# ai4co/rl4co

Hardware: NVIDIA H100
Metric: node-selections/sec TSP-100 AM rollout (higher is better)
Workload: dtype f32

## Files before the change

rl4co_b200/csrc/gemm_tf32x3.cu:

```cuda
#include "co_common.cuh"
#include "wgmma.cuh"

namespace co {

constexpr int GM = 128, GN = 128, GK = 32;
constexpr int TILE_BYTES = GM * GK * 4;
constexpr uint32_t SBO = 1024;
constexpr int KB128 = 4;
constexpr int STAGES = 3;
constexpr int GEMM_THREADS = 384;
constexpr int GEMM_SMEM = 2 * KB128 * TILE_BYTES + STAGES * 2 * TILE_BYTES;

__device__ __forceinline__ float4 split_hi(float4 v) {
  return make_float4(wg::rna_tf32(v.x), wg::rna_tf32(v.y), wg::rna_tf32(v.z), wg::rna_tf32(v.w));
}
__device__ __forceinline__ float4 sub4(float4 a, float4 b) { return make_float4(a.x - b.x, a.y - b.y, a.z - b.z, a.w - b.w); }

__global__ void split_tf32_kernel(const float* __restrict__ w, float* __restrict__ hi, float* __restrict__ lo, long n) {
  long i = (long)blockIdx.x * blockDim.x + threadIdx.x;
  if (i < n) {
    const float v = w[i], h = wg::rna_tf32(v);
    hi[i] = h;
    lo[i] = v - h;
  }
}

struct GemmArgs {
  const float* A; const float* Whi; const float* Wlo; float* C;
  const float* bias; const float* residual; const float* scale; const float* shift;
  int M, Nout, K, lda, ldc, ldr, relu, n_tiles;
};

__device__ __forceinline__ void epilogue_regs(const GemmArgs& g, const float (&d)[64], int m0, int n0, int lane) {
  const int q = lane & 3;
#pragma unroll
  for (int j = 0; j < 16; ++j) {
    const int n = n0 + 8 * j + 2 * q;
    if (n >= g.Nout) continue;
    float2 bs = make_float2(0.f, 0.f), sc = make_float2(1.f, 1.f), sh = bs;
    if (g.bias) bs = __ldg(reinterpret_cast<const float2*>(g.bias + n));
    if (g.scale) { sc = __ldg(reinterpret_cast<const float2*>(g.scale + n)); sh = __ldg(reinterpret_cast<const float2*>(g.shift + n)); }
#pragma unroll
    for (int half = 0; half < 2; ++half) {
      const int row = m0 + (lane >> 2) + 8 * half;
      if (row >= g.M) continue;
      float2 o = make_float2(d[4 * j + 2 * half] + bs.x, d[4 * j + 2 * half + 1] + bs.y);
      if (g.residual) {
        const float2 r = *reinterpret_cast<const float2*>(g.residual + (size_t)row * g.ldr + n);
        o.x += r.x; o.y += r.y;
      }
      if (g.relu) { o.x = fmaxf(o.x, 0.f); o.y = fmaxf(o.y, 0.f); }
      if (g.scale) { o.x = fmaf(o.x, sc.x, sh.x); o.y = fmaf(o.y, sc.y, sh.y); }
      *reinterpret_cast<float2*>(g.C + (size_t)row * g.ldc + n) = o;
    }
  }
}

template <bool WSTAT>
struct KBlock {
  float4 a[8];
  float4 h[WSTAT ? 1 : 8], l[WSTAT ? 1 : 8];
};

template <bool WSTAT>
__global__ void __launch_bounds__(GEMM_THREADS, 1) gemm_tf32x3_kernel(const GemmArgs g, int m_tiles, int groups) {
  extern __shared__ __align__(1024) unsigned char smem[];
  constexpr int STAGE_BYTES = (WSTAT ? 2 : 4) * TILE_BYTES;
  unsigned char* sW = smem;
  unsigned char* sRing = smem + (WSTAT ? 2 * KB128 * TILE_BYTES : 0);
  __shared__ __align__(8) uint64_t bars[2 * STAGES];

  const int tid = threadIdx.x, warp = tid >> 5, lane = tid & 31;
  const int n_tile = blockIdx.x % g.n_tiles, group = blockIdx.x / g.n_tiles;
  const int n0 = n_tile * GN;
  const int nkb = g.K / GK;
  const uint32_t bar0 = wg::s32(bars);
  auto FULL_B = [&](int s) { return bar0 + 8 * s; };
  auto EMPTY_B = [&](int s) { return bar0 + 8 * (STAGES + s); };

  if (tid == 0) {
    for (int s = 0; s < STAGES; ++s) { wg::bar_init(FULL_B(s), 128); wg::bar_init(EMPTY_B(s), 256); }
    wg::bar_init_fence();
  }
  if (WSTAT) {
    const int r8 = lane & 7, c4 = lane >> 3;
    for (int item = warp; item < KB128 * 32; item += GEMM_THREADS / 32) {
      const int kb = item >> 5, qq = item & 31;
      const int rg = qq >> 1, chunk = 4 * (qq & 1) + c4, row = 8 * rg + r8;
      const uint32_t soff = rg * SBO + r8 * 128 + ((chunk ^ r8) << 4);
      float4 h = make_float4(0.f, 0.f, 0.f, 0.f), l = h;
      if (n0 + row < g.Nout) {
        h = __ldg(reinterpret_cast<const float4*>(g.Whi + (size_t)(n0 + row) * g.K + kb * GK + chunk * 4));
        l = __ldg(reinterpret_cast<const float4*>(g.Wlo + (size_t)(n0 + row) * g.K + kb * GK + chunk * 4));
      }
      *reinterpret_cast<float4*>(sW + (2 * kb) * TILE_BYTES + soff) = h;
      *reinterpret_cast<float4*>(sW + (2 * kb + 1) * TILE_BYTES + soff) = l;
    }
    wg::fence_async();
  }
  __syncthreads();

  if (warp < 4) {
    const int r4 = lane >> 3, c8 = lane & 7;
    auto load = [&](int mt, int kb, auto& R) {
#pragma unroll
      for (int j = 0; j < 8; ++j) {
        const int lrow = 16 * j + 4 * warp + r4;
        const int row = mt * GM + lrow;
        R.a[j] = make_float4(0.f, 0.f, 0.f, 0.f);
        if (mt < m_tiles && row < g.M)
          R.a[j] = __ldg(reinterpret_cast<const float4*>(g.A + (size_t)row * g.lda + kb * GK + c8 * 4));
        if constexpr (!WSTAT) {
          R.h[j] = R.l[j] = make_float4(0.f, 0.f, 0.f, 0.f);
          if (mt < m_tiles && n0 + lrow < g.Nout) {
            R.h[j] = __ldg(reinterpret_cast<const float4*>(g.Whi + (size_t)(n0 + lrow) * g.K + kb * GK + c8 * 4));
            R.l[j] = __ldg(reinterpret_cast<const float4*>(g.Wlo + (size_t)(n0 + lrow) * g.K + kb * GK + c8 * 4));
          }
        }
      }
    };
    KBlock<WSTAT> R;
    KBlock<true> Rn;
    load(group, 0, R);
    uint32_t it = 0;
    for (int mt = group; mt < m_tiles; mt += groups) {
      for (int kb = 0; kb < nkb; ++kb, ++it) {
        auto load_next = [&](auto& dst) { if (kb + 1 < nkb) load(mt, kb + 1, dst); else load(mt + groups, 0, dst); };
        if constexpr (WSTAT) load_next(Rn);
        const int s = it % STAGES;
        wg::bar_wait(EMPTY_B(s), ((it / STAGES) & 1) ^ 1);
        unsigned char* st = sRing + s * STAGE_BYTES;
#pragma unroll
        for (int j = 0; j < 8; ++j) {
          const int lrow = 16 * j + 4 * warp + r4;
          const uint32_t soff = (lrow >> 3) * SBO + (lrow & 7) * 128 + ((c8 ^ (lrow & 7)) << 4);
          const float4 h = split_hi(R.a[j]);
          *reinterpret_cast<float4*>(st + soff) = h;
          *reinterpret_cast<float4*>(st + TILE_BYTES + soff) = sub4(R.a[j], h);
          if (!WSTAT) {
            *reinterpret_cast<float4*>(st + 2 * TILE_BYTES + soff) = R.h[j];
            *reinterpret_cast<float4*>(st + 3 * TILE_BYTES + soff) = R.l[j];
          }
        }
        wg::fence_async();
        wg::bar_arrive(FULL_B(s));
        if constexpr (WSTAT) R = Rn; else load_next(R);
      }
    }
  } else {
    const int cw = (warp - 4) >> 2, w4 = warp & 3;
    uint32_t it = 0;
    float d[64];
    for (int mt = group; mt < m_tiles; mt += groups) {
      for (int kb = 0; kb < nkb; ++kb, ++it) {
        const int s = it % STAGES;
        wg::bar_wait(FULL_B(s), (it / STAGES) & 1);
        const uint32_t ahi = wg::s32(sRing + s * STAGE_BYTES) + cw * 64 * 128, alo = ahi + TILE_BYTES;
        const uint32_t bhi = WSTAT ? wg::s32(sW + (2 * kb) * TILE_BYTES) : wg::s32(sRing + s * STAGE_BYTES + 2 * TILE_BYTES);
        const uint32_t blo = bhi + TILE_BYTES;
        wg::pin(d);
        wg::fence();
#pragma unroll
        for (int kk = 0; kk < GK / 8; ++kk) {
          const uint32_t off = kk * 32;
          wg::mma_ss_n128(d, wg::desc_sw128(ahi + off, SBO), wg::desc_sw128(bhi + off, SBO), (kb | kk) != 0);
          wg::mma_ss_n128(d, wg::desc_sw128(alo + off, SBO), wg::desc_sw128(bhi + off, SBO), 1);
          wg::mma_ss_n128(d, wg::desc_sw128(ahi + off, SBO), wg::desc_sw128(blo + off, SBO), 1);
        }
        wg::commit();
        if (kb > 0) {
          wg::wait<1>();
          wg::bar_arrive(EMPTY_B((it - 1) % STAGES));
        }
      }
      wg::wait<0>();
      wg::pin(d);
      wg::bar_arrive(EMPTY_B((it - 1) % STAGES));
      epilogue_regs(g, d, mt * GM + 64 * cw + 16 * w4, n0, lane);
    }
  }
}

}

using namespace co;

extern "C" int co_split_tf32(const float* w, float* hi, float* lo, long n, void* stream) {
  if (!w || !hi || !lo || n < 0) return fail(CO_ERR_BAD_ARG, "co_split_tf32: bad argument%s");
  if (n == 0) return CO_OK;
  split_tf32_kernel<<<(unsigned)((n + 255) / 256), 256, 0, (cudaStream_t)stream>>>(w, hi, lo, n);
  return check_launch("co_split_tf32");
}

extern "C" int co_gemm_tf32x3(const float* A, const float* Whi, const float* Wlo, float* C, const float* bias,
                              const float* residual, const float* scale, const float* shift, int M, int Nout, int K,
                              int lda, int ldc, int ldr, int relu, void* stream) {
  if (!A || !Whi || !Wlo || !C) return fail(CO_ERR_BAD_ARG, "co_gemm_tf32x3: null pointer%s");
  if (M < 0 || Nout <= 0 || K <= 0) return fail(CO_ERR_BAD_ARG, "co_gemm_tf32x3: bad shape%s");
  if ((K % GK) || (Nout % 4) || (lda % 4) || (ldc % 4) || (residual && (ldr % 4)))
    return fail(CO_ERR_UNSUPPORTED, "co_gemm_tf32x3: K %% 32, Nout %% 4 and 16-byte row strides required%s");
  if ((scale == nullptr) != (shift == nullptr)) return fail(CO_ERR_BAD_ARG, "co_gemm_tf32x3: scale and shift go together%s");
  if (((uintptr_t)A | (uintptr_t)Whi | (uintptr_t)Wlo | (uintptr_t)C | (uintptr_t)bias | (uintptr_t)residual |
       (uintptr_t)scale | (uintptr_t)shift) & 15)
    return fail(CO_ERR_BAD_ARG, "co_gemm_tf32x3: pointers must be 16-byte aligned%s");
  if (M == 0) return CO_OK;
  GemmArgs g{A, Whi, Wlo, C, bias, residual, scale, shift, M, Nout, K, lda, ldc, ldr, relu, (Nout + GN - 1) / GN};
  const int m_tiles = (M + GM - 1) / GM;
  if ((long)m_tiles * g.n_tiles > 0x7fffffffL) return fail(CO_ERR_UNSUPPORTED, "co_gemm_tf32x3: too many tiles%s");
  static PerDeviceOnce once;
  bool& configured = once.flag();
  if (!configured) {
    cudaError_t e = cudaFuncSetAttribute(gemm_tf32x3_kernel<true>, cudaFuncAttributeMaxDynamicSharedMemorySize, GEMM_SMEM);
    if (e == cudaSuccess)
      e = cudaFuncSetAttribute(gemm_tf32x3_kernel<false>, cudaFuncAttributeMaxDynamicSharedMemorySize, STAGES * 4 * TILE_BYTES);
    if (e != cudaSuccess) return fail(CO_ERR_CUDA, "co_gemm_tf32x3: smem attribute: %s", cudaGetErrorString(e));
    configured = true;
  }
  int groups = device_info().sm_count / g.n_tiles;
  if (groups < 1) groups = 1;
  if (groups > m_tiles) groups = m_tiles;
  if (K == GK * KB128)
    gemm_tf32x3_kernel<true><<<groups * g.n_tiles, GEMM_THREADS, GEMM_SMEM, (cudaStream_t)stream>>>(g, m_tiles, groups);
  else
    gemm_tf32x3_kernel<false><<<groups * g.n_tiles, GEMM_THREADS, STAGES * 4 * TILE_BYTES, (cudaStream_t)stream>>>(g, m_tiles, groups);
  return check_launch("co_gemm_tf32x3");
}
```

Baseline: 109.0 million.

## Overlap previous tile's epilogue with next tile's WGMMA k-blocks in static-weight GEMM

In the static-weight path, the consumer warpgroup copies the finished accumulator into a second register array. It then spreads that tile's epilogue stores across the four k-block iterations of the next M tile, so global stores run while asynchronous WGMMAs are in flight instead of after them. The cost is a second 64-float register array per thread, which raises register pressure and may cause spills. The loop is also fixed to KB128 k-blocks, which assumes K equals 128 in that path.

Measured after the change: 111.0 million (median of 6 runs). 1.9% higher.

```diff
diff --git a/rl4co_b200/csrc/gemm_tf32x3.cu b/rl4co_b200/csrc/gemm_tf32x3.cu
--- a/rl4co_b200/csrc/gemm_tf32x3.cu
+++ b/rl4co_b200/csrc/gemm_tf32x3.cu
@@ -31,10 +31,11 @@
   int M, Nout, K, lda, ldc, ldr, relu, n_tiles;
 };
 
+template <int JLO = 0, int JHI = 16>
 __device__ __forceinline__ void epilogue_regs(const GemmArgs& g, const float (&d)[64], int m0, int n0, int lane) {
   const int q = lane & 3;
 #pragma unroll
-  for (int j = 0; j < 16; ++j) {
+  for (int j = JLO; j < JHI; ++j) {
     const int n = n0 + 8 * j + 2 * q;
     if (n >= g.Nout) continue;
     float2 bs = make_float2(0.f, 0.f), sc = make_float2(1.f, 1.f), sh = bs;
@@ -149,34 +150,70 @@
     }
   } else {
     const int cw = (warp - 4) >> 2, w4 = warp & 3;
+    const int rows = 64 * cw + 16 * w4;
     uint32_t it = 0;
-    float d[64];
-    for (int mt = group; mt < m_tiles; mt += groups) {
-      for (int kb = 0; kb < nkb; ++kb, ++it) {
-        const int s = it % STAGES;
-        wg::bar_wait(FULL_B(s), (it / STAGES) & 1);
-        const uint32_t ahi = wg::s32(sRing + s * STAGE_BYTES) + cw * 64 * 128, alo = ahi + TILE_BYTES;
-        const uint32_t bhi = WSTAT ? wg::s32(sW + (2 * kb) * TILE_BYTES) : wg::s32(sRing + s * STAGE_BYTES + 2 * TILE_BYTES);
-        const uint32_t blo = bhi + TILE_BYTES;
-        wg::pin(d);
-        wg::fence();
-#pragma unroll
-        for (int kk = 0; kk < GK / 8; ++kk) {
-          const uint32_t off = kk * 32;
-          wg::mma_ss_n128(d, wg::desc_sw128(ahi + off, SBO), wg::desc_sw128(bhi + off, SBO), (kb | kk) != 0);
-          wg::mma_ss_n128(d, wg::desc_sw128(alo + off, SBO), wg::desc_sw128(bhi + off, SBO), 1);
-          wg::mma_ss_n128(d, wg::desc_sw128(ahi + off, SBO), wg::desc_sw128(blo + off, SBO), 1);
-        }
-        wg::commit();
-        if (kb > 0) {
-          wg::wait<1>();
-          wg::bar_arrive(EMPTY_B((it - 1) % STAGES));
-        }
+    auto kblock = [&](float (&d)[64], int kb) {
+      const int s = it % STAGES;
+      wg::bar_wait(FULL_B(s), (it / STAGES) & 1);
+      const uint32_t ahi = wg::s32(sRing + s * STAGE_BYTES) + cw * 64 * 128, alo = ahi + TILE_BYTES;
+      const uint32_t bhi = WSTAT ? wg::s32(sW + (2 * kb) * TILE_BYTES) : wg::s32(sRing + s * STAGE_BYTES + 2 * TILE_BYTES);
+      const uint32_t blo = bhi + TILE_BYTES;
+      wg::pin(d);
+      wg::fence();
+#pragma unroll
+      for (int kk = 0; kk < GK / 8; ++kk) {
+        const uint32_t off = kk * 32;
+        wg::mma_ss_n128(d, wg::desc_sw128(ahi + off, SBO), wg::desc_sw128(bhi + off, SBO), (kb | kk) != 0);
+        wg::mma_ss_n128(d, wg::desc_sw128(alo + off, SBO), wg::desc_sw128(bhi + off, SBO), 1);
+        wg::mma_ss_n128(d, wg::desc_sw128(ahi + off, SBO), wg::desc_sw128(blo + off, SBO), 1);
+      }
+      wg::commit();
+      ++it;
+    };
+    auto release_prev = [&]() {
+      wg::wait<1>();
+      wg::bar_arrive(EMPTY_B((it - 2) % STAGES));
+    };
+    if constexpr (WSTAT) {
+      float d[64], e[64];
+      int m0p = -1;
+      for (int mt = group; mt < m_tiles; mt += groups) {
+#pragma unroll
+        for (int kb = 0; kb < KB128; ++kb) {
+          if (kb == 0 && it > 0) {
+            wg::wait<0>();
+            wg::bar_arrive(EMPTY_B((it - 1) % STAGES));
+            wg::pin(d);
+#pragma unroll
+            for (int i = 0; i < 64; ++i) e[i] = d[i];
+          }
+          kblock(d, kb);
+          if (kb > 0) release_prev();
+          if (m0p >= 0) {
+            if (kb == 0) epilogue_regs<0, 4>(g, e, m0p, n0, lane);
+            if (kb == 1) epilogue_regs<4, 8>(g, e, m0p, n0, lane);
+            if (kb == 2) epilogue_regs<8, 12>(g, e, m0p, n0, lane);
+            if (kb == 3) epilogue_regs<12, 16>(g, e, m0p, n0, lane);
+          }
+        }
+        m0p = mt * GM + rows;
       }
       wg::wait<0>();
       wg::pin(d);
       wg::bar_arrive(EMPTY_B((it - 1) % STAGES));
-      epilogue_regs(g, d, mt * GM + 64 * cw + 16 * w4, n0, lane);
+      epilogue_regs(g, d, m0p, n0, lane);
+    } else {
+      float d[64];
+      for (int mt = group; mt < m_tiles; mt += groups) {
+        for (int kb = 0; kb < nkb; ++kb) {
+          kblock(d, kb);
+          if (kb > 0) release_prev();
+        }
+        wg::wait<0>();
+        wg::pin(d);
+        wg::bar_arrive(EMPTY_B((it - 1) % STAGES));
+        epilogue_regs(g, d, mt * GM + rows, n0, lane);
+      }
     }
   }
 }
```

## Use TMA-fed register-A wgmma kernel with overlapped epilogue for K=128 GEMM

Applied to the files above, without the earlier changes.

Adds a dedicated K=128 kernel. A single producer thread loads raw A tiles with TMA into a 6-deep ring, and consumer warpgroups split A into hi/lo TF32 fragments in registers and issue register-sourced wgmma. Producer registers are reduced and consumer registers raised via setmaxnreg. Two accumulator sets let the previous tile's epilogue be spread across the next tile's k-blocks. This removes the producer warps' global loads and shared-memory stores of split A. The cost is host-side tensor-map encoding on every call and higher register pressure.

Measured after the change: 108.9 million before, 114.8 million after (median of 6 runs). 5.4% higher.

```diff
diff --git a/rl4co_b200/csrc/gemm_tf32x3.cu b/rl4co_b200/csrc/gemm_tf32x3.cu
--- a/rl4co_b200/csrc/gemm_tf32x3.cu
+++ b/rl4co_b200/csrc/gemm_tf32x3.cu
@@ -1,3 +1,6 @@
+#include <cuda.h>
+#include <cudaTypedefs.h>
+
 #include "co_common.cuh"
 #include "wgmma.cuh"
 
@@ -8,8 +11,10 @@
 constexpr uint32_t SBO = 1024;
 constexpr int KB128 = 4;
 constexpr int STAGES = 3;
+constexpr int RING128 = 6;
 constexpr int GEMM_THREADS = 384;
-constexpr int GEMM_SMEM = 2 * KB128 * TILE_BYTES + STAGES * 2 * TILE_BYTES;
+constexpr int GEMM_SMEM = STAGES * 4 * TILE_BYTES;
+constexpr int GEMM128_SMEM = 2 * KB128 * TILE_BYTES + RING128 * TILE_BYTES;
 
 __device__ __forceinline__ float4 split_hi(float4 v) {
   return make_float4(wg::rna_tf32(v.x), wg::rna_tf32(v.y), wg::rna_tf32(v.z), wg::rna_tf32(v.w));
@@ -31,10 +36,11 @@
   int M, Nout, K, lda, ldc, ldr, relu, n_tiles;
 };
 
-__device__ __forceinline__ void epilogue_regs(const GemmArgs& g, const float (&d)[64], int m0, int n0, int lane) {
+__device__ __forceinline__ void epilogue_regs(const GemmArgs& g, const float (&d)[64], int m0, int n0, int lane,
+                                              int j0 = 0, int j1 = 16) {
   const int q = lane & 3;
 #pragma unroll
-  for (int j = 0; j < 16; ++j) {
+  for (int j = j0; j < j1; ++j) {
     const int n = n0 + 8 * j + 2 * q;
     if (n >= g.Nout) continue;
     float2 bs = make_float2(0.f, 0.f), sc = make_float2(1.f, 1.f), sh = bs;
@@ -56,18 +62,14 @@
   }
 }
 
-template <bool WSTAT>
 struct KBlock {
-  float4 a[8];
-  float4 h[WSTAT ? 1 : 8], l[WSTAT ? 1 : 8];
+  float4 a[8], h[8], l[8];
 };
 
-template <bool WSTAT>
 __global__ void __launch_bounds__(GEMM_THREADS, 1) gemm_tf32x3_kernel(const GemmArgs g, int m_tiles, int groups) {
   extern __shared__ __align__(1024) unsigned char smem[];
-  constexpr int STAGE_BYTES = (WSTAT ? 2 : 4) * TILE_BYTES;
-  unsigned char* sW = smem;
-  unsigned char* sRing = smem + (WSTAT ? 2 * KB128 * TILE_BYTES : 0);
+  constexpr int STAGE_BYTES = 4 * TILE_BYTES;
+  unsigned char* sRing = smem;
   __shared__ __align__(8) uint64_t bars[2 * STAGES];
 
   const int tid = threadIdx.x, warp = tid >> 5, lane = tid & 31;
@@ -82,7 +84,119 @@
     for (int s = 0; s < STAGES; ++s) { wg::bar_init(FULL_B(s), 128); wg::bar_init(EMPTY_B(s), 256); }
     wg::bar_init_fence();
   }
-  if (WSTAT) {
+  __syncthreads();
+
+  if (warp < 4) {
+    const int r4 = lane >> 3, c8 = lane & 7;
+    auto load = [&](int mt, int kb, auto& R) {
+#pragma unroll
+      for (int j = 0; j < 8; ++j) {
+        const int lrow = 16 * j + 4 * warp + r4;
+        const int row = mt * GM + lrow;
+        R.a[j] = make_float4(0.f, 0.f, 0.f, 0.f);
+        if (mt < m_tiles && row < g.M)
+          R.a[j] = __ldg(reinterpret_cast<const float4*>(g.A + (size_t)row * g.lda + kb * GK + c8 * 4));
+        R.h[j] = R.l[j] = make_float4(0.f, 0.f, 0.f, 0.f);
+        if (mt < m_tiles && n0 + lrow < g.Nout) {
+          R.h[j] = __ldg(reinterpret_cast<const float4*>(g.Whi + (size_t)(n0 + lrow) * g.K + kb * GK + c8 * 4));
+          R.l[j] = __ldg(reinterpret_cast<const float4*>(g.Wlo + (size_t)(n0 + lrow) * g.K + kb * GK + c8 * 4));
+        }
+      }
+    };
+    KBlock R;
+    load(group, 0, R);
+    uint32_t it = 0;
+    for (int mt = group; mt < m_tiles; mt += groups) {
+      for (int kb = 0; kb < nkb; ++kb, ++it) {
+        auto load_next = [&](auto& dst) { if (kb + 1 < nkb) load(mt, kb + 1, dst); else load(mt + groups, 0, dst); };
+        const int s = it % STAGES;
+        wg::bar_wait(EMPTY_B(s), ((it / STAGES) & 1) ^ 1);
+        unsigned char* st = sRing + s * STAGE_BYTES;
+#pragma unroll
+        for (int j = 0; j < 8; ++j) {
+          const int lrow = 16 * j + 4 * warp + r4;
+          const uint32_t soff = (lrow >> 3) * SBO + (lrow & 7) * 128 + ((c8 ^ (lrow & 7)) << 4);
+          const float4 h = split_hi(R.a[j]);
+          *reinterpret_cast<float4*>(st + soff) = h;
+          *reinterpret_cast<float4*>(st + TILE_BYTES + soff) = sub4(R.a[j], h);
+          *reinterpret_cast<float4*>(st + 2 * TILE_BYTES + soff) = R.h[j];
+          *reinterpret_cast<float4*>(st + 3 * TILE_BYTES + soff) = R.l[j];
+        }
+        wg::fence_async();
+        wg::bar_arrive(FULL_B(s));
+        load_next(R);
+      }
+    }
+  } else {
+    const int cw = (warp - 4) >> 2, w4 = warp & 3;
+    uint32_t it = 0;
+    float d[64];
+    for (int mt = group; mt < m_tiles; mt += groups) {
+      for (int kb = 0; kb < nkb; ++kb, ++it) {
+        const int s = it % STAGES;
+        wg::bar_wait(FULL_B(s), (it / STAGES) & 1);
+        const uint32_t ahi = wg::s32(sRing + s * STAGE_BYTES) + cw * 64 * 128, alo = ahi + TILE_BYTES;
+        const uint32_t bhi = wg::s32(sRing + s * STAGE_BYTES + 2 * TILE_BYTES);
+        const uint32_t blo = bhi + TILE_BYTES;
+        wg::pin(d);
+        wg::fence();
+#pragma unroll
+        for (int kk = 0; kk < GK / 8; ++kk) {
+          const uint32_t off = kk * 32;
+          wg::mma_ss_n128(d, wg::desc_sw128(ahi + off, SBO), wg::desc_sw128(bhi + off, SBO), (kb | kk) != 0);
+          wg::mma_ss_n128(d, wg::desc_sw128(alo + off, SBO), wg::desc_sw128(bhi + off, SBO), 1);
+          wg::mma_ss_n128(d, wg::desc_sw128(ahi + off, SBO), wg::desc_sw128(blo + off, SBO), 1);
+        }
+        wg::commit();
+        if (kb > 0) {
+          wg::wait<1>();
+          wg::bar_arrive(EMPTY_B((it - 1) % STAGES));
+        }
+      }
+      wg::wait<0>();
+      wg::pin(d);
+      wg::bar_arrive(EMPTY_B((it - 1) % STAGES));
+      epilogue_regs(g, d, mt * GM + 64 * cw + 16 * w4, n0, lane);
+    }
+  }
+}
+
+
+__device__ __forceinline__ void bar_expect_tx(uint32_t bar, uint32_t bytes) {
+  asm volatile("mbarrier.arrive.expect_tx.shared::cta.b64 _, [%0], %1;" ::"r"(bar), "r"(bytes) : "memory");
+}
+__device__ __forceinline__ void tma_load_2d(uint32_t dst, const CUtensorMap* map, int x, int y, uint32_t bar) {
+  asm volatile("cp.async.bulk.tensor.2d.shared::cluster.global.tile.mbarrier::complete_tx::bytes [%0], [%1, {%2, %3}], [%4];"
+               ::"r"(dst), "l"(reinterpret_cast<uint64_t>(map)), "r"(x), "r"(y), "r"(bar) : "memory");
+}
+
+#ifdef CO_GEMM_CLOCKS
+static __constant__ long long* co_gemm_clk;
+#define CO_GCLK(...) __VA_ARGS__
+#else
+#define CO_GCLK(...) ;
+#endif
+
+__global__ void __launch_bounds__(GEMM_THREADS, 1)
+    gemm_k128_kernel(const GemmArgs g, const __grid_constant__ CUtensorMap amap, int m_tiles, int groups) {
+  extern __shared__ __align__(1024) unsigned char smem[];
+  unsigned char* sW = smem;
+  unsigned char* sRing = smem + 2 * KB128 * TILE_BYTES;
+  __shared__ __align__(8) uint64_t bars[2 * RING128];
+  CO_GCLK(__shared__ long long issue_clk[RING128];)
+
+  const int tid = threadIdx.x, warp = tid >> 5, lane = tid & 31;
+  const int n_tile = blockIdx.x % g.n_tiles, group = blockIdx.x / g.n_tiles;
+  const int n0 = n_tile * GN;
+  const uint32_t bar0 = wg::s32(bars);
+  auto FULL_B = [&](int s) { return bar0 + 8 * s; };
+  auto EMPTY_B = [&](int s) { return bar0 + 8 * (RING128 + s); };
+
+  if (tid == 0) {
+    for (int s = 0; s < RING128; ++s) { wg::bar_init(FULL_B(s), 1); wg::bar_init(EMPTY_B(s), 256); }
+    wg::bar_init_fence();
+  }
+  {
     const int r8 = lane & 7, c4 = lane >> 3;
     for (int item = warp; item < KB128 * 32; item += GEMM_THREADS / 32) {
       const int kb = item >> 5, qq = item & 31;
@@ -101,89 +215,132 @@
   __syncthreads();
 
   if (warp < 4) {
-    const int r4 = lane >> 3, c8 = lane & 7;
-    auto load = [&](int mt, int kb, auto& R) {
-#pragma unroll
-      for (int j = 0; j < 8; ++j) {
-        const int lrow = 16 * j + 4 * warp + r4;
-        const int row = mt * GM + lrow;
-        R.a[j] = make_float4(0.f, 0.f, 0.f, 0.f);
-        if (mt < m_tiles && row < g.M)
-          R.a[j] = __ldg(reinterpret_cast<const float4*>(g.A + (size_t)row * g.lda + kb * GK + c8 * 4));
-        if constexpr (!WSTAT) {
-          R.h[j] = R.l[j] = make_float4(0.f, 0.f, 0.f, 0.f);
-          if (mt < m_tiles && n0 + lrow < g.Nout) {
-            R.h[j] = __ldg(reinterpret_cast<const float4*>(g.Whi + (size_t)(n0 + lrow) * g.K + kb * GK + c8 * 4));
-            R.l[j] = __ldg(reinterpret_cast<const float4*>(g.Wlo + (size_t)(n0 + lrow) * g.K + kb * GK + c8 * 4));
+    asm volatile("setmaxnreg.dec.sync.aligned.u32 24;");
+    if (tid == 0) {
+      CO_GCLK(long long c_empty = 0;)
+      uint32_t it = 0;
+      for (int mt = group; mt < m_tiles; mt += groups) {
+        for (int kb = 0; kb < KB128; ++kb, ++it) {
+          const int s = it % RING128;
+          CO_GCLK(const long long c0 = clock64();)
+          wg::bar_wait(EMPTY_B(s), ((it / RING128) & 1) ^ 1);
+          CO_GCLK(const long long c1 = clock64(); c_empty += c1 - c0; issue_clk[s] = c1;)
+          bar_expect_tx(FULL_B(s), TILE_BYTES);
+          tma_load_2d(wg::s32(sRing + s * TILE_BYTES), &amap, kb * GK, mt * GM, FULL_B(s));
+        }
+      }
+      CO_GCLK(co_gemm_clk[8 * blockIdx.x + 1] = c_empty;)
+    }
+  } else {
+    asm volatile("setmaxnreg.inc.sync.aligned.u32 240;");
+    const int cw = (warp - 4) >> 2, w4 = warp & 3, gq = lane >> 2;
+    const unsigned char* afrag = sRing + (8 * cw + 2 * w4) * SBO + gq * 128 + (lane & 3) * 4;
+    const int m_warp = 64 * cw + 16 * w4;
+    CO_GCLK(const bool rec = (tid == 128); long long c_lat = 0, c_full = 0, c_issue = 0, c_retire = 0, c_epi = 0, c_start = 0;
+            long long c_t = 0; int tiles = 0;)
+    uint32_t it = 0;
+    float d0[64], d1[64];
+    auto tile = [&](float (&dc)[64], float (&dp)[64], int mt, bool prev) {
+      CO_GCLK(++tiles;)
+#pragma unroll
+      for (int kb = 0; kb < KB128; ++kb, ++it) {
+        const int s = it % RING128;
+        CO_GCLK(c_t = clock64(); if (c_start == 0) c_start = c_t;)
+        wg::bar_wait(FULL_B(s), (it / RING128) & 1);
+        CO_GCLK(long long c = clock64(); c_full += c - c_t; c_lat += c - issue_clk[s]; c_t = c;)
+        const unsigned char* st = afrag + s * TILE_BYTES;
+        uint32_t bhi = wg::s32(sW + (2 * kb) * TILE_BYTES);
+        asm volatile("" : "+r"(bhi));
+        const uint32_t blo = bhi + TILE_BYTES;
+#pragma unroll
+        for (int kk = 0; kk < GK / 8; ++kk) {
+          uint32_t ah[4], al[4];
+#pragma unroll
+          for (int i = 0; i < 4; ++i) {
+            const float v = *reinterpret_cast<const float*>(st + (i & 1) * SBO + (((2 * kk + (i >> 1)) ^ gq) << 4));
+            const float h = wg::rna_tf32(v);
+            ah[i] = __float_as_uint(h);
+            al[i] = __float_as_uint(v - h);
           }
+          const uint32_t off = kk * 32;
+          if (kk == 0) wg::pin(dc);
+          wg::fence();
+          wg::mma_rs_n128(dc, ah, wg::desc_sw128(bhi + off, SBO), (kb | kk) != 0);
+          wg::mma_rs_n128(dc, al, wg::desc_sw128(bhi + off, SBO), 1);
+          wg::mma_rs_n128(dc, ah, wg::desc_sw128(blo + off, SBO), 1);
+          wg::commit();
+          if (kk == 0) {
+            CO_GCLK(c = clock64(); c_issue += c - c_t; c_t = c;)
+            if (kb > 0 || prev) {
+              wg::wait<1>();
+              wg::bar_arrive(EMPTY_B((it - 1) % RING128));
+            }
+            CO_GCLK(c = clock64(); c_retire += c - c_t; c_t = c;)
+          }
+        }
+        CO_GCLK(c = clock64(); c_issue += c - c_t; c_t = c;)
+        if (prev) {
+          if (kb == 0) wg::pin(dp);
+          epilogue_regs(g, dp, (mt - groups) * GM + m_warp, n0, lane, 4 * kb, 4 * kb + 4);
+          CO_GCLK(c = clock64(); c_epi += c - c_t;)
         }
       }
     };
-    KBlock<WSTAT> R;
-    KBlock<true> Rn;
-    load(group, 0, R);
-    uint32_t it = 0;
-    for (int mt = group; mt < m_tiles; mt += groups) {
-      for (int kb = 0; kb < nkb; ++kb, ++it) {
-        auto load_next = [&](auto& dst) { if (kb + 1 < nkb) load(mt, kb + 1, dst); else load(mt + groups, 0, dst); };
-        if constexpr (WSTAT) load_next(Rn);
-        const int s = it % STAGES;
-        wg::bar_wait(EMPTY_B(s), ((it / STAGES) & 1) ^ 1);
-        unsigned char* st = sRing + s * STAGE_BYTES;
-#pragma unroll
-        for (int j = 0; j < 8; ++j) {
-          const int lrow = 16 * j + 4 * warp + r4;
-          const uint32_t soff = (lrow >> 3) * SBO + (lrow & 7) * 128 + ((c8 ^ (lrow & 7)) << 4);
-          const float4 h = split_hi(R.a[j]);
-          *reinterpret_cast<float4*>(st + soff) = h;
-          *reinterpret_cast<float4*>(st + TILE_BYTES + soff) = sub4(R.a[j], h);
-          if (!WSTAT) {
-            *reinterpret_cast<float4*>(st + 2 * TILE_BYTES + soff) = R.h[j];
-            *reinterpret_cast<float4*>(st + 3 * TILE_BYTES + soff) = R.l[j];
-          }
-        }
-        wg::fence_async();
-        wg::bar_arrive(FULL_B(s));
-        if constexpr (WSTAT) R = Rn; else load_next(R);
-      }
-    }
-  } else {
-    const int cw = (warp - 4) >> 2, w4 = warp & 3;
-    uint32_t it = 0;
-    float d[64];
-    for (int mt = group; mt < m_tiles; mt += groups) {
-      for (int kb = 0; kb < nkb; ++kb, ++it) {
-        const int s = it % STAGES;
-        wg::bar_wait(FULL_B(s), (it / STAGES) & 1);
-        const uint32_t ahi = wg::s32(sRing + s * STAGE_BYTES) + cw * 64 * 128, alo = ahi + TILE_BYTES;
-        const uint32_t bhi = WSTAT ? wg::s32(sW + (2 * kb) * TILE_BYTES) : wg::s32(sRing + s * STAGE_BYTES + 2 * TILE_BYTES);
-        const uint32_t blo = bhi + TILE_BYTES;
-        wg::pin(d);
-        wg::fence();
-#pragma unroll
-        for (int kk = 0; kk < GK / 8; ++kk) {
-          const uint32_t off = kk * 32;
-          wg::mma_ss_n128(d, wg::desc_sw128(ahi + off, SBO), wg::desc_sw128(bhi + off, SBO), (kb | kk) != 0);
-          wg::mma_ss_n128(d, wg::desc_sw128(alo + off, SBO), wg::desc_sw128(bhi + off, SBO), 1);
-          wg::mma_ss_n128(d, wg::desc_sw128(ahi + off, SBO), wg::desc_sw128(blo + off, SBO), 1);
-        }
-        wg::commit();
-        if (kb > 0) {
-          wg::wait<1>();
-          wg::bar_arrive(EMPTY_B((it - 1) % STAGES));
-        }
-      }
+    auto last = [&](float (&dl)[64], int mt) {
       wg::wait<0>();
-      wg::pin(d);
-      wg::bar_arrive(EMPTY_B((it - 1) % STAGES));
-      epilogue_regs(g, d, mt * GM + 64 * cw + 16 * w4, n0, lane);
-    }
-  }
+      CO_GCLK(const long long c = clock64(); c_retire += c - c_t; c_t = c;)
+      wg::pin(dl);
+      epilogue_regs(g, dl, mt * GM + m_warp, n0, lane);
+    };
+    int mt = group;
+    if (mt < m_tiles) {
+      tile(d0, d1, mt, false);
+      for (;;) {
+        if (mt + groups >= m_tiles) { last(d0, mt); break; }
+        mt += groups;
+        tile(d1, d0, mt, true);
+        if (mt + groups >= m_tiles) { last(d1, mt); break; }
+        mt += groups;
+        tile(d0, d1, mt, true);
+      }
+    }
+    CO_GCLK(if (rec) {
+      const long long c = clock64();
+      long long* o = co_gemm_clk + 8 * blockIdx.x;
+      o[0] = tiles; o[2] = c_lat; o[3] = c_full; o[4] = c_issue; o[5] = c_retire; o[6] = c_epi + (c - c_t); o[7] = c - c_start;
+    })
+  }
+}
+
+static int encode_a_map(CUtensorMap* map, const float* A, int M, int K, int lda) {
+  static const PFN_cuTensorMapEncodeTiled_v12000 encode = []() -> PFN_cuTensorMapEncodeTiled_v12000 {
+    void* fn = nullptr;
+    cudaDriverEntryPointQueryResult q;
+    if (cudaGetDriverEntryPointByVersion("cuTensorMapEncodeTiled", &fn, 12000, cudaEnableDefault, &q) != cudaSuccess ||
+        q != cudaDriverEntryPointSuccess)
+      return nullptr;
+    return reinterpret_cast<PFN_cuTensorMapEncodeTiled_v12000>(fn);
+  }();
+  if (!encode) return fail(CO_ERR_CUDA, "co_gemm_tf32x3: cuTensorMapEncodeTiled is not available%s");
+  const cuuint64_t dims[2] = {(cuuint64_t)K, (cuuint64_t)M};
+  const cuuint64_t strides[1] = {(cuuint64_t)lda * sizeof(float)};
+  const cuuint32_t box[2] = {GK, GM}, estr[2] = {1, 1};
+  const CUresult r = encode(map, CU_TENSOR_MAP_DATA_TYPE_FLOAT32, 2, const_cast<float*>(A), dims, strides, box, estr,
+                            CU_TENSOR_MAP_INTERLEAVE_NONE, CU_TENSOR_MAP_SWIZZLE_128B, CU_TENSOR_MAP_L2_PROMOTION_L2_256B,
+                            CU_TENSOR_MAP_FLOAT_OOB_FILL_NONE);
+  if (r != CUDA_SUCCESS) return fail(CO_ERR_CUDA, "co_gemm_tf32x3: cuTensorMapEncodeTiled failed%s (CUresult %lld)", "", (long long)r);
+  return CO_OK;
 }
 
 }
 
 using namespace co;
+
+#ifdef CO_GEMM_CLOCKS
+extern "C" int co_gemm_clocks_set(void* buf) {
+  return cudaMemcpyToSymbol(co::co_gemm_clk, &buf, sizeof(buf)) == cudaSuccess ? 0 : 1;
+}
+#endif
 
 extern "C" int co_split_tf32(const float* w, float* hi, float* lo, long n, void* stream) {
   if (!w || !hi || !lo || n < 0) return fail(CO_ERR_BAD_ARG, "co_split_tf32: bad argument%s");
@@ -195,33 +352,36 @@
 extern "C" int co_gemm_tf32x3(const float* A, const float* Whi, const float* Wlo, float* C, const float* bias,
                               const float* residual, const float* scale, const float* shift, int M, int Nout, int K,
                               int lda, int ldc, int ldr, int relu, void* stream) {
-  if (!A || !Whi || !Wlo || !C) return fail(CO_ERR_BAD_ARG, "co_gemm_tf32x3: null pointer%s");
   if (M < 0 || Nout <= 0 || K <= 0) return fail(CO_ERR_BAD_ARG, "co_gemm_tf32x3: bad shape%s");
   if ((K % GK) || (Nout % 4) || (lda % 4) || (ldc % 4) || (residual && (ldr % 4)))
     return fail(CO_ERR_UNSUPPORTED, "co_gemm_tf32x3: K %% 32, Nout %% 4 and 16-byte row strides required%s");
   if ((scale == nullptr) != (shift == nullptr)) return fail(CO_ERR_BAD_ARG, "co_gemm_tf32x3: scale and shift go together%s");
+  if (M == 0) return CO_OK;
+  if (!A || !Whi || !Wlo || !C) return fail(CO_ERR_BAD_ARG, "co_gemm_tf32x3: null pointer%s");
   if (((uintptr_t)A | (uintptr_t)Whi | (uintptr_t)Wlo | (uintptr_t)C | (uintptr_t)bias | (uintptr_t)residual |
        (uintptr_t)scale | (uintptr_t)shift) & 15)
     return fail(CO_ERR_BAD_ARG, "co_gemm_tf32x3: pointers must be 16-byte aligned%s");
-  if (M == 0) return CO_OK;
   GemmArgs g{A, Whi, Wlo, C, bias, residual, scale, shift, M, Nout, K, lda, ldc, ldr, relu, (Nout + GN - 1) / GN};
   const int m_tiles = (M + GM - 1) / GM;
   if ((long)m_tiles * g.n_tiles > 0x7fffffffL) return fail(CO_ERR_UNSUPPORTED, "co_gemm_tf32x3: too many tiles%s");
   static PerDeviceOnce once;
   bool& configured = once.flag();
   if (!configured) {
-    cudaError_t e = cudaFuncSetAttribute(gemm_tf32x3_kernel<true>, cudaFuncAttributeMaxDynamicSharedMemorySize, GEMM_SMEM);
+    cudaError_t e = cudaFuncSetAttribute(gemm_k128_kernel, cudaFuncAttributeMaxDynamicSharedMemorySize, GEMM128_SMEM);
     if (e == cudaSuccess)
-      e = cudaFuncSetAttribute(gemm_tf32x3_kernel<false>, cudaFuncAttributeMaxDynamicSharedMemorySize, STAGES * 4 * TILE_BYTES);
+      e = cudaFuncSetAttribute(gemm_tf32x3_kernel, cudaFuncAttributeMaxDynamicSharedMemorySize, GEMM_SMEM);
     if (e != cudaSuccess) return fail(CO_ERR_CUDA, "co_gemm_tf32x3: smem attribute: %s", cudaGetErrorString(e));
     configured = true;
   }
   int groups = device_info().sm_count / g.n_tiles;
   if (groups < 1) groups = 1;
   if (groups > m_tiles) groups = m_tiles;
-  if (K == GK * KB128)
-    gemm_tf32x3_kernel<true><<<groups * g.n_tiles, GEMM_THREADS, GEMM_SMEM, (cudaStream_t)stream>>>(g, m_tiles, groups);
-  else
-    gemm_tf32x3_kernel<false><<<groups * g.n_tiles, GEMM_THREADS, STAGES * 4 * TILE_BYTES, (cudaStream_t)stream>>>(g, m_tiles, groups);
+  if (K == GK * KB128) {
+    CUtensorMap amap;
+    if (int rc = encode_a_map(&amap, A, M, K, lda)) return rc;
+    gemm_k128_kernel<<<groups * g.n_tiles, GEMM_THREADS, GEMM128_SMEM, (cudaStream_t)stream>>>(g, amap, m_tiles, groups);
+  } else {
+    gemm_tf32x3_kernel<<<groups * g.n_tiles, GEMM_THREADS, GEMM_SMEM, (cudaStream_t)stream>>>(g, m_tiles, groups);
+  }
   return check_launch("co_gemm_tf32x3");
 }
```
